# widgital/python-audio-tools

Hardware: AMD Instinct MI355X
Metric: FLAC-8 encode frames/s (4096-sample 44.1k stereo) at 1/2/4/8 GPUs; bit-exact (higher is better)
Workload: dtype int32 residuals / f64 LPC analysis (s16 PCM in); 1 GPU; FLAC-8 batch encode, 1024 tracks x 64 frames x 4096 samples per GPU, 44.1 kHz 16-bit stereo, PCM and .flac images in HBM; tracks_per_gpu=1024, frames_per_track=64, block_size=4096, preset=FLAC-8 (-l 12 -m -e -R 6), parallelism=dp1 (tracks sharded per GPU, weak scaling)

## Files before the change

### python-audio-tools_amd/csrc/engine.hip

```cpp
#include "handle_lock.h"
#include "host_common.h"
#include <hip/hip_runtime.h>

#include <sched.h>

#include <algorithm>
#include <array>
#include <cmath>
#include <condition_variable>
#include <cstdio>
#include <cstdlib>
#include <cstring>
#include <deque>
#include <functional>
#include <future>
#include <map>
#include <memory>
#include <mutex>
#include <string>
#include <thread>
#include <vector>

#include "../../include/atgpu.h"
#include "crc_common.h"
#include "flac_dev.h"
#include "launch.h"
#include "md5_cpu.h"
#include "ogg_demux.h"
#include "ogg_mux.h"

namespace {

thread_local ErrSlot g_err;
#define HIP_TRY(expr) ATG_HIP_TRY(g_err, expr, #expr)

const char kVendor[] = "Python Audio Tools 2.22alpha1";

const int kNumTimed = 8;
const char *kTimedNames[kNumTimed] = {"lpc_analyze", "subframe_search", "frame_decide",
                                      "track_scan",  "frame_pack",      "track_md5",
                                      "stream_header", "total"};
const char *kOggTimedNames[4] = {"ogg_plan", "ogg_pages", "ogg_split", "ogg_crc"};

void build_crc_tables(uint32_t t16[4][256], uint32_t *t8, uint16_t adv[24][16],
                      uint16_t advq[kCrcQ][6][16])
{
    crc_build_tables<16>(0x8005u, &t16[0][0], 4);
    crc_build_tables<8>(0x07u, t8, 1);
    crc_build_advance<16>(t16[0], &adv[0][0], 24);
    for (int i = 0; i < 16; ++i)
        advq[0][0][i] = adv[2][i];
    for (int q = 1; q < kCrcQ; ++q)
        for (int i = 0; i < 16; ++i)
            advq[q][0][i] = (uint16_t)crc_advance<16>(adv[2], advq[q - 1][0][i]);
    for (int q = 0; q < kCrcQ; ++q)
        for (int s = 1; s < 6; ++s)
            crc_square<16>(advq[q][s - 1], advq[q][s]);
}

}

namespace {
struct Plan;
struct HostJob;
}

struct EncSlot {
    DevBuf frames, tracks, order, coef, shift, est, sub, fdesc, tout, err;
    DevBuf rice_big, scratch;
    DevBuf slow;
    hipStream_t s_aux = nullptr;
    hipEvent_t ev[2 * kNumTimed] = {};
    hipEvent_t ev_tables = nullptr, ev_pack = nullptr, ev_done = nullptr;
    std::shared_ptr<Plan> plan;
    const Plan *uploaded = nullptr;
    hipEvent_t ev_reuse = nullptr;
    bool reuse_pending = false;
    TrackOut *tout_h = nullptr;
    size_t tout_cap = 0;
    FrameDesc *fdesc_h = nullptr;
    size_t fdesc_cap = 0;
    uint32_t *err_h = nullptr;
    size_t err_cap = 0;
    bool want_fdesc = false;
    bool end_pending = false;
    const void *pend_pcm = nullptr;
    int pend_fmt = 0;
    uint8_t *pend_out = nullptr;
    bool pend_split = false;
    atg_status end_status = ATG_OK;
    std::string end_error;
    bool md5_host = false;
    uint8_t *hpcm = nullptr;
    size_t hpcm_cap = 0;
    DevBuf dpack;
    uint8_t *hmd5 = nullptr;
    size_t hmd5_cap = 0;
    DevBuf md5in;
    hipEvent_t ev_hpcm = nullptr;
    std::vector<std::future<void>> hash_jobs;
    bool rolled = false;
    uint32_t roll_parts = 0, roll_done = 0;
    bool busy = false;
    bool done = false;
    bool host = false;
    uint64_t ticket = 0;
    atg_status status = ATG_OK;
    std::string error;
    float times[kNumTimed] = {};
};



constexpr uint64_t kEncSlots = 3;
constexpr uint64_t kMaxSlots = 32;
static_assert(kMaxSlots <= kRollMax, "one rolled launch covers every slot");
constexpr uint64_t kRollMinDepth = 4;

constexpr uint64_t kHostStages = kEncSlots + 1;

constexpr size_t kResultCopy = 8192;

struct HostStage {
    DevBuf d_pcm, d_img, d_pack, d_off;
    uint8_t *p_in = nullptr, *p_out = nullptr;
    size_t p_in_cap = 0, p_out_cap = 0;
    uint64_t *p_off = nullptr;
    size_t p_off_cap = 0;
    hipEvent_t ev_h2d = nullptr;
    hipEvent_t ev_packed = nullptr;
    hipEvent_t ev_d2h = nullptr;
};

struct HashPool {
    std::vector<std::thread> th;
    std::mutex mu;
    std::condition_variable cv;
    std::deque<std::packaged_task<void()>> q;
    bool stop = false;
    explicit HashPool(unsigned n)
    {
        for (unsigned i = 0; i < n; ++i)
            th.emplace_back([this] {
                for (;;) {
                    std::packaged_task<void()> job;
                    {
                        std::unique_lock<std::mutex> lk(mu);
                        cv.wait(lk, [this] { return stop || !q.empty(); });
                        if (q.empty())
                            return;
                        job = std::move(q.front());
                        q.pop_front();
                    }
                    job();
                }
            });
    }
    std::future<void> submit(std::function<void()> f)
    {
        std::packaged_task<void()> job(std::move(f));
        std::future<void> fut = job.get_future();
        {
            std::lock_guard<std::mutex> lk(mu);
            q.push_back(std::move(job));
        }
        cv.notify_one();
        return fut;
    }
    ~HashPool()
    {
        {
            std::lock_guard<std::mutex> lk(mu);
            stop = true;
        }
        cv.notify_all();
        for (std::thread &t : th)
            t.join();
    }
};

struct atg_engine {
    std::recursive_mutex mu;
    int device = 0;
    uint32_t flags = 0;
    std::unique_ptr<HashPool> pool;
    bool sync_call = false;
    hipStream_t s_main = nullptr;
    hipStream_t s_pack = nullptr;
    EncSlot slot[kMaxSlots];
    uint64_t depth = kEncSlots;
    bool depth_user = false;
    hipStream_t s_md5 = nullptr;
    std::deque<EncSlot *> roll_q;
    DevBuf windows;
    HostStage hs[kHostStages];
    hipStream_t s_h2d = nullptr, s_d2h = nullptr;
    hipStream_t s_hpack = nullptr;
    uint64_t chunk_bytes = 512ull << 20;
    std::deque<std::unique_ptr<HostJob>> hjobs;
    std::deque<std::pair<HostJob *, size_t>> hflight;
    HostJob *hcopy_job = nullptr;
    size_t hcopy_chunk = 0;
    uint64_t hseq = 0;
    uint64_t next_hjob = 1;
    std::map<uint32_t, uint32_t> win_off;
    std::vector<double> win_host;
    size_t win_uploaded = 0;
    hipEvent_t ev_win = nullptr;
    float times[kNumTimed] = {};
    bool have_times = false;
    uint64_t next_ticket = 1;
    std::vector<uint8_t> plan_key;
    std::shared_ptr<Plan> plan_cached;
    DevBuf ogg_stage, ogg_tmpl, ogg_hp, ogg_trk, ogg_frm, ogg_pgoff, ogg_out, ogg_pages;
    DevBuf ogg_pcm, ogg_img;
    const uint32_t *ogg_crc = nullptr, *ogg_adv = nullptr;
    hipEvent_t ogg_ev[5] = {};
    float ogg_times[4] = {};
    bool ogg_last = false;
};

namespace {

struct Plan {
    FlacParams p;
    std::vector<FrameInfo> frames;
    std::vector<TrackInfo> tracks;
    std::vector<uint32_t> track_frame_pos;
    std::vector<uint32_t> order;
    uint64_t frame_bound = 0;
    uint64_t out_bytes = 0;
    uint32_t n_reg_prefix = 0;
    bool big = false;
    uint32_t big_nmax = 0;
    uint32_t big_porder = 0;
    bool frames_only = false;
};

const uint32_t kBigGrid = 1024;

uint64_t big_row_bytes(const Plan &pl) { return ((uint64_t)pl.big_nmax * 4u + 255u) & ~255ull; }

uint64_t big_slot_bytes(const Plan &pl)
{
    return big_row_bytes(pl) + (16ull << pl.big_porder);
}

uint32_t qlp_precision_for(uint32_t n)
{
    return n <= 192 ? 7 : n <= 384 ? 8 : n <= 576 ? 9 : n <= 1152 ? 10 : n <= 2304 ? 11
         : n <= 4608 ? 12 : 13;
}

atg_status make_plan(const atg_flac_options *o, const atg_track *tracks, uint32_t n_tracks,
                     uint32_t channels, uint32_t bps, uint32_t rate, Plan &pl,
                     bool frames_only = false, uint32_t index_base = 0,
                     const uint32_t *index_bases = nullptr)
{
    if (!o)
        return g_err.fail(ATG_ERR_INVALID, "options is NULL");
    if (channels < 1 || channels > 8)
        return g_err.fail(ATG_ERR_INVALID, "channels must be 1..8");
    if (bps < 4 || bps > 24)
        return g_err.fail(ATG_ERR_UNSUPPORTED, "bits_per_sample must be 4..24 on the GPU path");
    if (o->block_size == 0)
        return g_err.fail(ATG_ERR_INVALID, "block_size must be > 0");
    if (o->block_size > ATG_BIG_MAX_BLOCK)
        return g_err.fail(ATG_ERR_UNSUPPORTED, "block_size > 65535 cannot be framed");
    if (o->max_lpc_order > ATG_MAX_LPC)
        return g_err.fail(ATG_ERR_INVALID, "max_lpc_order must be <= 32");
    if (o->max_residual_partition_order > ATG_BIG_MAX_PORDER)
        return g_err.fail(ATG_ERR_INVALID, "max_residual_partition_order must be <= 15");
    if (o->padding_size > 0xFFFFFFu)
        return g_err.fail(ATG_ERR_INVALID, "padding_size must fit in 24 bits");
    if (rate == 0)
        return g_err.fail(ATG_ERR_INVALID, "sample_rate must be > 0");
    FlacParams &p = pl.p;
    std::memset(&p, 0, sizeof(p));
    p.block_size = o->block_size;
    p.max_lpc_order = o->max_lpc_order;
    p.max_porder = o->max_residual_partition_order;
    p.qlp_precision = qlp_precision_for(o->block_size);
    p.max_rice = bps <= 16 ? 14 : 30;
    p.mid_side = o->mid_side != 0;
    p.adaptive_mid_side = o->adaptive_mid_side != 0;
    p.exhaustive = o->exhaustive_model_search != 0;
    p.try_verbatim = !o->disable_verbatim_subframes;
    p.try_constant = !o->disable_constant_subframes;
    p.try_fixed = !o->disable_fixed_subframes;
    p.try_lpc = !(o->disable_lpc_subframes || o->max_lpc_order == 0);
    p.channels = channels;
    p.bps = bps;
    p.sample_rate = rate;
    p.n_cand = (channels == 2 && (p.mid_side || p.adaptive_mid_side)) ? 4 : channels;
    p.n_tracks = n_tracks;
    const uint32_t M = p.max_lpc_order;
    p.coef_row = std::max<uint32_t>(2, (M + 1u) & ~1u);
    p.coef_stride = std::max<uint32_t>(1, M) * p.coef_row;
    p.padding_size = o->padding_size;
    p.header_bytes = frames_only ? 0u : 4 + 4 + 34 + 4 + 4 + 29 + 4 + 4 + o->padding_size;
    pl.frames_only = frames_only;

    const uint64_t B = o->block_size;
    const uint64_t nsub = channels;

    pl.tracks.resize(n_tracks);
    std::vector<uint32_t> lens;
    std::vector<uint32_t> owner;
    for (uint32_t t = 0; t < n_tracks; ++t) {
        const atg_track &tr = tracks[t];
        TrackInfo &ti = pl.tracks[t];
        ti.pcm_start = tr.pcm_offset;
        ti.pcm_frames = tr.pcm_frames;
        ti.first_pos = (uint32_t)lens.size();
        if (tr.frame_sizes) {
            uint64_t sum = 0;
            for (uint64_t k = 0; k < tr.n_frame_sizes; ++k) {
                const uint32_t n = tr.frame_sizes[k];
                if (n == 0 || n > ATG_BIG_MAX_BLOCK)
                    return g_err.fail(n ? ATG_ERR_UNSUPPORTED : ATG_ERR_INVALID,
                                "explicit frame sizes must be 1..65535");
                sum += n;
                lens.push_back(n);
                owner.push_back(t);
            }
            if (sum != tr.pcm_frames)
                return g_err.fail(ATG_ERR_INVALID, "frame sizes do not sum to pcm_frames");
        } else {
            for (uint64_t done = 0; done < tr.pcm_frames; done += B) {
                lens.push_back((uint32_t)std::min<uint64_t>(B, tr.pcm_frames - done));
                owner.push_back(t);
            }
        }
        ti.n_frames = (uint32_t)(lens.size() - ti.first_pos);
        if (lens.size() > 0x7FFFFFFFull)
            return g_err.fail(ATG_ERR_INVALID, "too many frames in one batch");
    }
    const size_t nfr = lens.size();
    pl.order.resize(nfr);
    pl.frames.resize(nfr);
    pl.track_frame_pos.resize(n_tracks);
    size_t n_full = 0;
    for (size_t i = 0; i < nfr; ++i)
        n_full += lens[i] == B ? 1 : 0;
    size_t id_full = 0, id_other = n_full;
    std::vector<uint64_t> start(n_tracks, 0);
    std::vector<uint32_t> idx(n_tracks, 0);
    for (size_t i = 0; i < nfr; ++i) {
        const uint32_t t = owner[i];
        const size_t id = lens[i] == B ? id_full++ : id_other++;
        pl.order[i] = (uint32_t)id;
        FrameInfo &f = pl.frames[id];
        f.pcm_start = pl.tracks[t].pcm_start + start[t];
        f.n = lens[i];
        f.track = t;
        f.index = (index_bases ? index_bases[t] : index_base) + idx[t]++;
        f.win_off = 0;
        start[t] += lens[i];
    }
    uint32_t maxn = 0;
    for (size_t i = 0; i < nfr; ++i)
        maxn = std::max(maxn, lens[i]);
    const uint64_t nb = std::max<uint64_t>(B, maxn);
    uint64_t fb = 16 + nsub * ((8 + 32 + nb * (bps + 1) + 7) / 8) + 2;
    pl.big = nb > ATG_MAX_BLOCK || p.max_porder > ATG_MAX_PORDER;
    if (!p.try_verbatim)
        fb = pl.big ? 2 * fb + 120 * 1024 : std::max<uint64_t>(fb, 120 * 1024);
    pl.frame_bound = fb;
    p.frame_bound = (uint32_t)fb;
    p.frame_lds_words = (uint32_t)((fb + 3) / 4 + 2);
    if (!pl.big && p.frame_lds_words * 4ull > 128 * 1024)
        return g_err.fail(ATG_ERR_UNSUPPORTED, "frame image exceeds the pack kernel's LDS budget");
    if (pl.big) {
        pl.big_nmax = maxn;
        pl.big_porder = 0;
        for (size_t i = 0; i < nfr; ++i) {
            const uint32_t tz = (uint32_t)__builtin_ctz(lens[i]);
            pl.big_porder = std::max(pl.big_porder, std::min<uint32_t>(p.max_porder, tz));
        }
    }
    uint64_t out = 0;
    for (uint32_t t = 0; t < n_tracks; ++t) {
        TrackInfo &ti = pl.tracks[t];
        pl.track_frame_pos[t] = ti.first_pos;
        ti.out_base = out;
        out += p.header_bytes + (uint64_t)ti.n_frames * fb;
        out = (out + 15) & ~15ull;
    }
    p.n_frames = (uint32_t)pl.frames.size();
    pl.out_bytes = out;
    pl.n_reg_prefix = 0;
    if (channels == 2 && p.n_cand == 4 && bps <= 16 && B == ATG_MAX_BLOCK && !pl.big)
        while (pl.n_reg_prefix < p.n_frames && pl.frames[pl.n_reg_prefix].n == ATG_MAX_BLOCK &&
               (pl.frames[pl.n_reg_prefix].pcm_start & 3u) == 0)
            pl.n_reg_prefix++;
    return ATG_OK;
}

void tukey(uint32_t N, double *w)
{
    const double alpha = 0.5;
    const unsigned window1 = (unsigned)(alpha * (N - 1)) / 2;
    const unsigned window2 = (unsigned)((N - 1) * (1.0 - (alpha / 2.0)));
    for (unsigned n = 0; n < N; n++) {
        if (n <= window1)
            w[n] = 0.5 * (1.0 + std::cos(M_PI * (((2 * n) / (alpha * (N - 1))) - 1.0)));
        else if (n <= window2)
            w[n] = 1.0;
        else
            w[n] = 0.5 * (1.0 + std::cos(M_PI * (((2.0 * n) / (alpha * (N - 1))) -
                                                 (2.0 / alpha) + 1.0)));
    }
}

atg_status prepare_windows(atg_engine *e, Plan &pl, hipStream_t s)
{
    if (!pl.p.try_lpc)
        return ATG_OK;
    const uint32_t M = pl.p.max_lpc_order;
    for (FrameInfo &f : pl.frames) {
        if (f.n <= M + 1)
            continue;
        auto it = e->win_off.find(f.n);
        if (it == e->win_off.end()) {
            const uint32_t off = (uint32_t)e->win_host.size();
            e->win_host.resize(off + f.n);
            tukey(f.n, e->win_host.data() + off);
            it = e->win_off.emplace(f.n, off).first;
        }
        f.win_off = it->second;
    }
    if (e->win_host.size() != e->win_uploaded) {
        const size_t need = e->win_host.size() * sizeof(double) + 64;
        if (need > e->windows.cap && e->windows.p)
            HIP_TRY(hipDeviceSynchronize());
        HIP_TRY(e->windows.ensure(need));
        HIP_TRY(hipMemcpyAsync(e->windows.p, e->win_host.data(),
                               e->win_host.size() * sizeof(double), hipMemcpyHostToDevice,
                               s));
        e->win_uploaded = e->win_host.size();
        if (!e->ev_win)
            HIP_TRY(hipEventCreateWithFlags(&e->ev_win, hipEventDisableTiming));
        HIP_TRY(hipEventRecord(e->ev_win, s));
    } else if (e->ev_win) {
        HIP_TRY(hipStreamWaitEvent(s, e->ev_win, 0));
    }
    return ATG_OK;
}

void par_memcpy(void *dst, const void *src, size_t n, unsigned nt)
{
    const size_t kMin = 8u << 20;
    if (n < kMin || nt < 2) {
        std::memcpy(dst, src, n);
        return;
    }
    nt = (unsigned)std::min<size_t>(nt, n / (kMin / 4));
    std::vector<std::thread> th;
    const size_t part = (n / nt + 4095) & ~(size_t)4095;
    for (unsigned i = 0; i < nt; ++i) {
        const size_t a = (size_t)i * part;
        if (a >= n)
            break;
        const size_t len = std::min(part, n - a);
        th.emplace_back([=] { std::memcpy((uint8_t *)dst + a, (const uint8_t *)src + a, len); });
    }
    for (auto &t : th)
        t.join();
}

bool is_pinned(const void *p)
{
    if (!p)
        return false;
    hipPointerAttribute_t a;
    if (hipPointerGetAttributes(&a, p) != hipSuccess) {
        (void)hipGetLastError();
        return false;
    }
    return a.type == hipMemoryTypeHost;
}

template <class T>
hipError_t ensure_pinned(T *&p, size_t &cap, size_t n)
{
    if (p && n <= cap)
        return hipSuccess;
    if (p)
        (void)hipHostFree(p);
    p = nullptr;
    cap = 0;
    const size_t want = std::max<size_t>(n, 16);
    hipError_t e = hipHostMalloc((void **)&p, want * sizeof(T), hipHostMallocDefault);
    if (e == hipSuccess)
        cap = want;
    return e;
}

atg_status batch_end_queue(atg_engine *e, EncSlot &sl, hipEvent_t after);

atg_status batch_end(atg_engine *e, EncSlot &sl, hipEvent_t after)
{
    sl.end_pending = false;
    const atg_status st = batch_end_queue(e, sl, after);
    if (st != ATG_OK) {
        sl.end_status = st;
        sl.end_error = g_err.msg;
    }
    return st;
}

atg_status batch_end_queue(atg_engine *e, EncSlot &sl, hipEvent_t after)
{
    const Plan &pl = *sl.plan;
    const FlacParams &p = pl.p;
    const size_t nf = pl.frames.size(), nt = pl.tracks.size();
    const TrackInfo *dtr = (const TrackInfo *)sl.tracks.p;
    TrackOut *dto = (TrackOut *)sl.tout.p;
    uint32_t *derr = (uint32_t *)sl.err.p;
    hipEvent_t *ev = sl.ev;
    hipStream_t q = sl.rolled ? e->s_md5 : sl.s_aux;
    if (sl.rolled) {
        if (!pl.frames_only)
            HIP_TRY(launch_track_md5_finish(p, sl.pend_pcm, sl.pend_fmt, dtr, dto, q));
    } else if (sl.pend_split && !pl.frames_only) {
        if (after)
            HIP_TRY(hipStreamWaitEvent(q, after, 0));
        HIP_TRY(launch_track_md5(p, sl.pend_pcm, sl.pend_fmt, dtr, dto, 1, q));
    }
    HIP_TRY(hipEventRecord(ev[2 * 5 + 1], q));
    HIP_TRY(hipStreamWaitEvent(q, sl.ev_pack, 0));
    HIP_TRY(hipEventRecord(ev[12], q));
    if (!pl.frames_only)
        HIP_TRY(launch_stream_header(p, dtr, dto, sl.pend_out, q));
    HIP_TRY(hipEventRecord(ev[13], q));
    HIP_TRY(hipEventRecord(ev[15], q));
    for (size_t o = 0, nb = nt * sizeof(TrackOut); o < nb; o += kResultCopy)
        HIP_TRY(hipMemcpyAsync((uint8_t *)sl.tout_h + o, (const uint8_t *)dto + o,
                               std::min<size_t>(kResultCopy, nb - o), hipMemcpyDeviceToHost, q));
    if (sl.want_fdesc && nf)
        HIP_TRY(hipMemcpyAsync(sl.fdesc_h, sl.fdesc.p, nf * sizeof(FrameDesc),
                               hipMemcpyDeviceToHost, q));
    HIP_TRY(hipMemcpyAsync(sl.err_h, derr, sizeof(uint32_t), hipMemcpyDeviceToHost, q));
    HIP_TRY(hipEventRecord(sl.ev_done, q));
    return ATG_OK;
}

atg_status ensure_aux_stream(EncSlot &sl);

atg_status ensure_roll_streams(atg_engine *e)
{
    if (e->s_md5)
        return ATG_OK;
    int prio_lo = 0, prio_hi = 0;
    HIP_TRY(hipDeviceGetStreamPriorityRange(&prio_lo, &prio_hi));
    HIP_TRY(hipStreamCreateWithPriority(&e->s_md5, hipStreamNonBlocking, prio_hi));
    return ATG_OK;
}

atg_status roll_step(atg_engine *e, hipEvent_t after, EncSlot *only)
{
    MdRollArgs a;
    std::memset(&a, 0, sizeof(a));
    std::vector<EncSlot *> starting, finished;
    uint32_t wg = 0;
    for (EncSlot *sl : e->roll_q) {
        if (only && sl != only)
            continue;
        const FlacParams &p = sl->plan->p;
        MdRollBatch &b = a.b[a.n++];
        b.pcm = sl->pend_pcm;
        b.tracks = (const TrackInfo *)sl->tracks.p;
        b.tout = (TrackOut *)sl->tout.p;
        b.n_tracks = p.n_tracks;
        b.channels = p.channels;
        b.bps = p.bps;
        b.fmt = (uint32_t)sl->pend_fmt;
        b.wg0 = wg;
        b.parts = sl->roll_parts;
        b.part = sl->roll_done;
        b.part_end = only ? sl->roll_parts : sl->roll_done + 1u;
        wg += (p.n_tracks + 63u) / 64u;
        if (b.part == 0)
            starting.push_back(sl);
        sl->roll_done = b.part_end;
        if (sl->roll_done == sl->roll_parts)
            finished.push_back(sl);
    }
    if (!a.n)
        return ATG_OK;
    if (after)
        HIP_TRY(hipStreamWaitEvent(e->s_md5, after, 0));
    for (EncSlot *sl : starting)
        HIP_TRY(hipEventRecord(sl->ev[2 * 5], e->s_md5));
    HIP_TRY(launch_track_md5_roll(a, e->s_md5));
    for (EncSlot *sl : finished) {
        e->roll_q.erase(std::find(e->roll_q.begin(), e->roll_q.end(), sl));
        const atg_status st = batch_end(e, *sl, nullptr);
        if (st != ATG_OK)
            return st;
    }
    return ATG_OK;
}

void drain_slot(atg_engine *e, EncSlot &sl)
{
    (void)hipStreamSynchronize(e->s_main);
    for (hipStream_t q : {e->s_pack, e->s_md5, sl.s_aux})
        if (q)
            (void)hipStreamSynchronize(q);
}

unsigned host_hash_threads()
{
    unsigned n = std::max(1u, std::thread::hardware_concurrency());
    cpu_set_t cs;
    if (sched_getaffinity(0, sizeof(cs), &cs) == 0)
        n = std::max(1, CPU_COUNT(&cs));
    if (FILE *f = std::fopen("/sys/fs/cgroup/cpu.max", "r")) {
        char q[32] = {0};
        unsigned long per = 0;
        if (std::fscanf(f, "%31s %lu", q, &per) == 2 && std::strcmp(q, "max") != 0 && per)
            n = std::min<unsigned>(n, std::max(1ul, std::strtoul(q, nullptr, 10) / per));
        std::fclose(f);
    }
    return std::min(n, 32u);
}

constexpr size_t kHashGroup = md5cpu::kMultiLanes;

bool want_host_md5(atg_engine *e, const Plan &pl, int fmt, bool md5_early)
{
    const FlacParams &p = pl.p;
    if (pl.frames_only || md5_early || p.bps < 8 || p.bps % 8 || pl.tracks.empty())
        return false;
    if (e->flags & ATG_ENGINE_MD5_GPU)
        return false;
    if (e->flags & ATG_ENGINE_MD5_HOST)
        return true;
    const uint64_t bb = p.bps / 8, cs = fmt == ATG_PCM_S16 ? 2 : 4;
    uint64_t maxb = 0, tot = 0;
    for (const TrackInfo &t : pl.tracks) {
        const uint64_t b = t.pcm_frames * p.channels * bb;
        maxb = std::max(maxb, b);
        tot += b;
    }
    (void)cs;
    const double gpu_ms = (double)maxb / 64.0 * 0.8e-3;
    const unsigned th = host_hash_threads();
    const uint64_t groups = (pl.tracks.size() + kHashGroup - 1) / kHashGroup;
    const double hash_ms = md5cpu::multi_simd()
                               ? (double)tot / (double)std::min<uint64_t>(th, groups) / 6e6
                               : (double)tot / (th * 450e3);
    const double host_ms = hash_ms + (double)tot / 40e6;
    return gpu_ms > 40.0 && host_ms < gpu_ms;
}

atg_status start_host_md5(atg_engine *e, EncSlot &sl, const Plan &pl, const void *d_pcm, int fmt)
{
    const FlacParams &p = pl.p;
    const size_t nt = pl.tracks.size();
    const uint64_t cs = fmt == ATG_PCM_S16 ? 2 : 4;
    const uint32_t bb = p.bps / 8;
    for (std::future<void> &f : sl.hash_jobs)
        f.wait();
    sl.hash_jobs.clear();
    std::vector<uint64_t> off(nt), len(nt);
    uint64_t total = 0;
    for (size_t t = 0; t < nt; ++t) {
        len[t] = pl.tracks[t].pcm_frames * p.channels * bb;
        off[t] = total;
        total += (len[t] + 15u) & ~15ull;
    }
    HIP_TRY(ensure_pinned(sl.hpcm, sl.hpcm_cap, (size_t)std::max<uint64_t>(total, 1)));
    HIP_TRY(ensure_pinned(sl.hmd5, sl.hmd5_cap, 16 * nt));
    HIP_TRY(sl.md5in.ensure(16 * nt));
    HIP_TRY(sl.dpack.ensure((size_t)std::max<uint64_t>(total, 1)));
    if (!sl.ev_hpcm)
        HIP_TRY(hipEventCreateWithFlags(&sl.ev_hpcm, hipEventDisableTiming));
    for (size_t t = 0; t < nt; ++t) {
        const TrackInfo &ti = pl.tracks[t];
        HIP_TRY(launch_md5_pack((const uint8_t *)d_pcm + ti.pcm_start * p.channels * cs,
                                fmt == ATG_PCM_S16, ti.pcm_frames * p.channels, bb,
                                (uint8_t *)sl.dpack.p + off[t], sl.s_aux));
    }
    if (total)
        HIP_TRY(hipMemcpyAsync(sl.hpcm, sl.dpack.p, total, hipMemcpyDeviceToHost, sl.s_aux));
    HIP_TRY(hipEventRecord(sl.ev_hpcm, sl.s_aux));
    if (!e->pool)
        e->pool.reset(new HashPool(host_hash_threads()));
    const hipEvent_t ev = sl.ev_hpcm;
    for (size_t g0 = 0; g0 < nt; g0 += kHashGroup) {
        const int n = (int)std::min<size_t>(kHashGroup, nt - g0);
        std::array<const uint8_t *, kHashGroup> src{};
        std::array<uint64_t, kHashGroup> bytes{};
        for (int i = 0; i < n; ++i) {
            src[i] = sl.hpcm + off[g0 + i];
            bytes[i] = len[g0 + i];
        }
        uint8_t(*dst)[16] = (uint8_t(*)[16])(sl.hmd5 + 16 * g0);
        sl.hash_jobs.push_back(e->pool->submit([=] {
            (void)hipEventSynchronize(ev);
            md5cpu::hash_bytes_multi(src.data(), bytes.data(), n, dst);
        }));
    }
    return ATG_OK;
}

atg_status finish_host_md5(EncSlot &sl)
{
    for (std::future<void> &f : sl.hash_jobs)
        f.wait();
    sl.hash_jobs.clear();
    const size_t nt = sl.plan->tracks.size();
    if (nt) {
        HIP_TRY(hipMemcpyAsync(sl.md5in.p, sl.hmd5, 16 * nt, hipMemcpyHostToDevice, sl.s_aux));
        HIP_TRY(launch_put_md5((TrackOut *)sl.tout.p, (const uint8_t *)sl.md5in.p, (uint32_t)nt,
                               sl.s_aux));
    }
    return ATG_OK;
}

atg_status enqueue_batch(atg_engine *e, EncSlot &sl, const std::shared_ptr<Plan> &plp,
                         const void *d_pcm, int fmt, uint8_t *d_out, uint64_t out_cap,
                         bool want_fdesc, hipEvent_t wait_before = nullptr, bool pipelined = false,
                         bool md5_early = false)
{
    Plan &pl = *plp;
    FlacParams &p = pl.p;
    if (pl.out_bytes > out_cap)
// ... 1659 lines not shown
```

### python-audio-tools_amd/csrc/flac_lpc.hip

```cpp
#include <hip/hip_runtime.h>
#include <math.h>
#include <stdint.h>

#include "flac_dev.h"
#include "launch.h"
#include "pcm_read.h"
#include "residual.h"
#include "wave.h"

#pragma clang fp contract(off)


__device__ __forceinline__ int32_t d2i_x86(double x)
{
    if (!(x > -2147483649.0 && x < 2147483648.0))
        return INT32_MIN;
    return (int32_t)x;
}

template <int LAGS>
__device__ __forceinline__ void quantize_store(const double (&lp)[LAGS],
                                               int order, int prec,
                                               int16_t *__restrict__ q, uint32_t row,
                                               int8_t *__restrict__ shift_out)
{
    double l = 2.2250738585072014e-308;
#pragma unroll
    for (int i = 0; i < LAGS; ++i) {
        if (i < order) {
            const double a = fabs(lp[i]);
            l = a > l ? a : l;
        }
    }
    int log2cmax;
    frexp(l, &log2cmax);
    int shift = (prec - 1) - (log2cmax - 1) - 1;
    shift = shift < -16 ? -16 : shift;
    shift = shift > 15 ? 15 : shift;
    const int qmax = (1 << (prec - 1)) - 1;
    const int qmin = -(1 << (prec - 1));
    double err = 0.0;
#pragma unroll
    for (int i = 0; i < LAGS; ++i) {
        if (i < order) {
            if (shift >= 0)
                err += lp[i] * (double)(1 << shift);
            else
                err += lp[i] / (double)(1 << -shift);
            const int32_t ei = d2i_x86(round(err));
            q[i] = (int16_t)(ei < qmin ? qmin : (ei > qmax ? qmax : ei));
            err -= (double)ei;
        }
    }
    for (uint32_t i = (uint32_t)order; i < row; ++i)
        q[i] = 0;
    *shift_out = (int8_t)(shift >= 0 ? shift : 0);
}

template <int MODE, typename T, int K>
__device__ __forceinline__ void autocorr(const T *__restrict__ src, const double *__restrict__ win,
                                         uint32_t ch, uint32_t cand, uint32_t n_loop,
                                         uint32_t nlast, uint32_t n_max, double (&acc)[K],
                                         double (&hist)[K])
{
    int32_t sv[K];
    double wv[K];
#pragma unroll
    for (int u = 0; u < K; ++u) {
        const uint32_t j = min((uint32_t)u, nlast);
        sv[u] = cand_at<MODE>(src, j, ch, cand);
        wv[u] = win[j];
    }
    for (uint32_t j0 = 0; j0 < n_max; j0 += K) {
        double xv[K];
#pragma unroll
        for (int u = 0; u < K; ++u)
            xv[u] = (j0 + (uint32_t)u < n_loop) ? (double)sv[u] * wv[u] : 0.0;
#pragma unroll
        for (int u = 0; u < K; ++u) {
            const uint32_t j = min(j0 + K + (uint32_t)u, nlast);
            sv[u] = cand_at<MODE>(src, j, ch, cand);
            wv[u] = win[j];
        }
#pragma unroll
        for (int u = 0; u < K; ++u) {
            const double x = xv[u];
            hist[u] = x;
#pragma unroll
            for (int L = 0; L < K; ++L) {
                const double prod = hist[(u - L + K) % K] * x;
                acc[L] = acc[L] + prod;
            }
        }
    }
}

template <int K, bool VEC4>
__device__ __forceinline__ void autocorr_ms16(const uint32_t *__restrict__ pairs,
                                              const double *__restrict__ win, uint32_t cand,
                                              uint32_t N, double (&acc)[K], double (&hist)[K])
{
    const uint32_t wts = cand == 0u ? 0x00000001u : cand == 1u ? 0x00010000u
                       : cand == 2u ? 0x00010001u : 0xFFFF0001u;
    const int gsh = cand == 2u ? 1 : 0;
    const uint32_t nfull = N / K * K;
    uint32_t j0 = 0;
    if (VEC4) {
        const uint4 *__restrict__ q4 = (const uint4 *)pairs;
        for (; j0 + 4u * K <= N; j0 += 4u * K) {
            uint32_t pv[4 * K];
#pragma unroll
            for (int i = 0; i < K; ++i) {
                const uint4 v = q4[(j0 >> 2) + (uint32_t)i];
                pv[4 * i] = v.x;
                pv[4 * i + 1] = v.y;
                pv[4 * i + 2] = v.z;
                pv[4 * i + 3] = v.w;
            }
#pragma unroll
            for (int i = 0; i < 4 * K; ++i)
                asm volatile("" : "+v"(pv[i]));
#pragma unroll
            for (int sub = 0; sub < 4; ++sub) {
                double xv[K];
#pragma unroll
                for (int u = 0; u < K; ++u) {
                    const int v = __builtin_amdgcn_sdot2(
                        __builtin_bit_cast(short2_t, pv[sub * K + u]),
                        __builtin_bit_cast(short2_t, wts), 0, false);
                    xv[u] = (double)(v >> gsh) * win[j0 + (uint32_t)(sub * K + u)];
                }
#pragma unroll
                for (int u = 0; u < K; ++u) {
                    const double x = xv[u];
                    hist[u] = x;
#pragma unroll
                    for (int L = 0; L < K; ++L) {
                        const double prod = hist[(u - L + K) % K] * x;
                        acc[L] = acc[L] + prod;
                    }
                }
            }
        }
    }
    for (; j0 < nfull; j0 += K) {
        double xv[K];
#pragma unroll
        for (int u = 0; u < K; ++u) {
            const int v = __builtin_amdgcn_sdot2(__builtin_bit_cast(short2_t, pairs[j0 + u]),
                                                 __builtin_bit_cast(short2_t, wts), 0, false);
            xv[u] = (double)(v >> gsh) * win[j0 + u];
        }
#pragma unroll
        for (int u = 0; u < K; ++u) {
            const double x = xv[u];
            hist[u] = x;
#pragma unroll
            for (int L = 0; L < K; ++L) {
                const double prod = hist[(u - L + K) % K] * x;
                acc[L] = acc[L] + prod;
            }
        }
    }
    if (j0 < N) {
        double xv[K];
#pragma unroll
        for (int u = 0; u < K; ++u) {
            const uint32_t j = min(j0 + (uint32_t)u, N - 1u);
            const int v = __builtin_amdgcn_sdot2(__builtin_bit_cast(short2_t, pairs[j]),
                                                 __builtin_bit_cast(short2_t, wts), 0, false);
            xv[u] = j0 + (uint32_t)u < N ? (double)(v >> gsh) * win[j] : 0.0;
        }
#pragma unroll
        for (int u = 0; u < K; ++u) {
            const double x = xv[u];
            hist[u] = x;
#pragma unroll
            for (int L = 0; L < K; ++L) {
                const double prod = hist[(u - L + K) % K] * x;
                acc[L] = acc[L] + prod;
            }
        }
    }
}

template <typename T, int LAGS>
__global__ __launch_bounds__(64) void k_lpc_analyze(
    FlacParams p, const T *__restrict__ pcm,
    const FrameInfo *__restrict__ frames, const double *__restrict__ windows,
    int16_t *__restrict__ coef_tab, int8_t *__restrict__ shift_tab,
    uint8_t *__restrict__ est_tab)
{
    constexpr int K = LAGS + 1;
    const uint32_t fpw = 64u / p.n_cand;
    const uint32_t fl = threadIdx.x / p.n_cand;
    const uint32_t cand = threadIdx.x - fl * p.n_cand;
    const uint32_t f = blockIdx.x * fpw + fl;
    const bool ms = (p.n_cand == 4u) && (p.channels == 2u);
    const bool active = fl < fpw && f < p.n_frames;
    const FrameInfo fi = frames[active ? f : 0u];
    const int M = (int)p.max_lpc_order;
    const uint32_t N = active ? fi.n : 0u;
    const bool do_lpc = active && N > (uint32_t)M + 1u;
    const uint32_t n_loop = do_lpc ? N : 0u;
    const uint32_t n_max = wave_max_u32(n_loop);
    if (n_max == 0u)
        return;

    double acc[K];
    double hist[K];
#pragma unroll
    for (int k = 0; k < K; ++k) {
        acc[k] = 0.0;
        hist[k] = 0.0;
    }
    const double *__restrict__ win = windows + fi.win_off;
    const T *__restrict__ src = pcm + fi.pcm_start * p.channels;
    const uint32_t nlast = n_loop ? n_loop - 1u : 0u;
    const int mode = pcm_mode(pcm, ms);
    const uint32_t n_first = uniform_u32(do_lpc ? N : 0u);
    const bool uniform_n = wave_all(!active || (do_lpc ? N : 0u) == n_first) && n_first > 0u;
    if (mode == PCM_MS16 && uniform_n) {
        const double *__restrict__ wu =
            windows + uniform_u32(active ? fi.win_off : 0u);
        const bool al16 = wave_all(((uintptr_t)src & 15u) == 0u);
        if (al16)
            autocorr_ms16<K, true>((const uint32_t *)src, wu, cand, n_first, acc, hist);
        else
            autocorr_ms16<K, false>((const uint32_t *)src, wu, cand, n_first, acc, hist);
    } else switch (mode) {
    case PCM_MS16:
        autocorr<PCM_MS16, T, K>(src, win, p.channels, cand, n_loop, nlast, n_max, acc, hist);
        break;
    case PCM_MS:
        autocorr<PCM_MS, T, K>(src, win, p.channels, cand, n_loop, nlast, n_max, acc, hist);
        break;
    default:
        autocorr<PCM_CH, T, K>(src, win, p.channels, cand, n_loop, nlast, n_max, acc, hist);
    }
    if (!do_lpc)
        return;

    const size_t sub = (size_t)f * p.n_cand + cand;
    int16_t *__restrict__ qout = coef_tab + sub * p.coef_stride;
    int8_t *__restrict__ sout = shift_tab + sub * (size_t)M;
    const int prec = (int)p.qlp_precision;

    double prev[LAGS], cur[LAGS], errv[LAGS];
#pragma unroll
    for (int k = 0; k < LAGS; ++k) {
        prev[k] = 0.0;
        cur[k] = 0.0;
        errv[k] = 0.0;
    }
    double k0 = acc[1] / acc[0];
    cur[0] = k0;
    errv[0] = acc[0] * (1.0 - (k0 * k0));
    quantize_store<LAGS>(cur, 1, prec, qout, p.coef_row, sout);
#pragma unroll
    for (int i = 1; i < LAGS; ++i) {
        if (i < M) {
#pragma unroll
            for (int j = 0; j < LAGS; ++j)
                prev[j] = cur[j];
            double q = acc[i + 1];
#pragma unroll
            for (int j = 0; j < LAGS; ++j)
                if (j < i)
                    q -= (prev[j] * acc[i - j]);
            const double kk = q / errv[i - 1];
#pragma unroll
            for (int j = 0; j < LAGS; ++j)
                if (j < i)
                    cur[j] = prev[j] - (kk * prev[i - j - 1]);
            cur[i] = kk;
            errv[i] = errv[i - 1] * (1.0 - (kk * kk));
            quantize_store<LAGS>(cur, i + 1, prec, qout + i * p.coef_row, p.coef_row,
                                 sout + i);
        }
    }

    if (!p.exhaustive) {
        const double ln2 = 0.69314718055994530942;
        const double error_scale = (ln2 * ln2) / ((double)N * 2.0);
        int best = 0;
        double best_bits = 1.7976931348623157e308;
        bool done = false;
#pragma unroll
        for (int i = 0; i < LAGS; ++i) {
            if (i < M && !done) {
                const int order = i + 1;
                if (errv[i] > 0.0) {
                    const unsigned header = (unsigned)order * (p.bps + p.qlp_precision);
                    double bpr = log(errv[i] * error_scale) / (ln2 * 2);
                    bpr = bpr > 0.0 ? bpr : 0.0;
                    const double est = (double)header + bpr * (double)(N - (unsigned)order);
                    if (est < best_bits) {
                        best = order;
                        best_bits = est;
                    }
                } else {
                    best = order;
                    done = true;
                }
            }
        }
        est_tab[sub] = (uint8_t)best;
    }
}

template <typename T, int LAGS>
static hipError_t launch_t(const FlacParams &p, const T *pcm, const FrameInfo *frames,
                           const double *windows, int16_t *coef_tab,
                           int8_t *shift_tab, uint8_t *est_tab, hipStream_t s)
{
    const uint32_t fpw = 64u / p.n_cand;
    dim3 grid((p.n_frames + fpw - 1u) / fpw);
    hipLaunchKernelGGL((k_lpc_analyze<T, LAGS>), grid, dim3(64), 0, s, p, pcm,
                       frames, windows, coef_tab, shift_tab, est_tab);
    return hipGetLastError();
}

template <typename T>
static hipError_t launch_lags(const FlacParams &p, const T *pcm,
                              const FrameInfo *frames, const double *windows,
                              int16_t *coef_tab, int8_t *shift_tab,
                              uint8_t *est_tab, hipStream_t s)
{
    const uint32_t M = p.max_lpc_order;
    if (M <= 8)
        return launch_t<T, 8>(p, pcm, frames, windows, coef_tab, shift_tab, est_tab, s);
    if (M <= 12)
        return launch_t<T, 12>(p, pcm, frames, windows, coef_tab, shift_tab, est_tab, s);
    return launch_t<T, ATG_MAX_LPC>(p, pcm, frames, windows, coef_tab, shift_tab,
                                    est_tab, s);
}

hipError_t launch_lpc_analyze(const FlacParams &p, const void *pcm, int fmt,
                              const FrameInfo *frames, const double *windows,
                              int16_t *coef_tab, int8_t *shift_tab,
                              uint8_t *est_tab, hipStream_t s)
{
    if (p.max_lpc_order == 0 || !p.try_lpc || p.n_frames == 0)
        return hipSuccess;
    if (fmt == 0)
        return launch_lags<int16_t>(p, (const int16_t *)pcm, frames, windows,
                                    coef_tab, shift_tab, est_tab, s);
    return launch_lags<int32_t>(p, (const int32_t *)pcm, frames, windows,
                                coef_tab, shift_tab, est_tab, s);
}
```

Before: 8.620 million frames/s.

## Skip window multiply and fuse autocorrelation FMAs inside flat Tukey window region

The host now records, in a slot just before each window, the contiguous range where the Tukey window equals 1.0. Inside that range the autocorrelation kernels skip the window load and multiply and accumulate with FMA instead of a separate multiply and add. This holds bit-exactly only when the products of integer samples are exact in double, which the LPC_FMA_MAX_BITS check on bps is meant to guarantee. The cost is extra per-group branching and a shifted window layout.

```diff
diff --git a/python-audio-tools_amd/csrc/engine.hip b/python-audio-tools_amd/csrc/engine.hip
--- a/python-audio-tools_amd/csrc/engine.hip
+++ b/python-audio-tools_amd/csrc/engine.hip
@@ -25,6 +25,7 @@
 #include "crc_common.h"
 #include "flac_dev.h"
 #include "launch.h"
+#include "lpc_flat.h"
 #include "md5_cpu.h"
 #include "ogg_demux.h"
 #include "ogg_mux.h"
@@ -423,9 +424,12 @@
             continue;
         auto it = e->win_off.find(f.n);
         if (it == e->win_off.end()) {
-            const uint32_t off = (uint32_t)e->win_host.size();
+            const uint32_t off = (uint32_t)e->win_host.size() + 1u;
             e->win_host.resize(off + f.n);
             tukey(f.n, e->win_host.data() + off);
+            const WinFlat wf = window_flat_run(e->win_host.data() + off, f.n);
+            static_assert(sizeof(WinFlat) == sizeof(double), "WinFlat fills one window slot");
+            memcpy(e->win_host.data() + off - 1, &wf, sizeof wf);
             it = e->win_off.emplace(f.n, off).first;
         }
         f.win_off = it->second;
diff --git a/python-audio-tools_amd/csrc/flac_lpc.hip b/python-audio-tools_amd/csrc/flac_lpc.hip
--- a/python-audio-tools_amd/csrc/flac_lpc.hip
+++ b/python-audio-tools_amd/csrc/flac_lpc.hip
@@ -4,6 +4,7 @@
 
 #include "flac_dev.h"
 #include "launch.h"
+#include "lpc_flat.h"
 #include "pcm_read.h"
 #include "residual.h"
 #include "wave.h"
@@ -60,8 +61,8 @@
 template <int MODE, typename T, int K>
 __device__ __forceinline__ void autocorr(const T *__restrict__ src, const double *__restrict__ win,
                                          uint32_t ch, uint32_t cand, uint32_t n_loop,
-                                         uint32_t nlast, uint32_t n_max, double (&acc)[K],
-                                         double (&hist)[K])
+                                         uint32_t nlast, uint32_t n_max, uint2 flat,
+                                         double (&acc)[K], double (&hist)[K])
 {
     int32_t sv[K];
     double wv[K];
@@ -71,34 +72,38 @@
         sv[u] = cand_at<MODE>(src, j, ch, cand);
         wv[u] = win[j];
     }
+    bool fused = false;
     for (uint32_t j0 = 0; j0 < n_max; j0 += K) {
         double xv[K];
 #pragma unroll
-        for (int u = 0; u < K; ++u)
-            xv[u] = (j0 + (uint32_t)u < n_loop) ? (double)sv[u] * wv[u] : 0.0;
+        for (int u = 0; u < K; ++u) {
+            const bool in = j0 + (uint32_t)u < n_loop;
+            if (fused)
+                xv[u] = in ? (double)sv[u] : 0.0;
+            else
+                xv[u] = in ? (double)sv[u] * wv[u] : 0.0;
+        }
+        const bool fused_next = wave_all(n_loop == 0u || group_flat<K>(j0 + K, flat.x, flat.y));
 #pragma unroll
         for (int u = 0; u < K; ++u) {
             const uint32_t j = min(j0 + K + (uint32_t)u, nlast);
             sv[u] = cand_at<MODE>(src, j, ch, cand);
-            wv[u] = win[j];
-        }
-#pragma unroll
-        for (int u = 0; u < K; ++u) {
-            const double x = xv[u];
-            hist[u] = x;
-#pragma unroll
-            for (int L = 0; L < K; ++L) {
-                const double prod = hist[(u - L + K) % K] * x;
-                acc[L] = acc[L] + prod;
-            }
-        }
+            if (!fused_next)
+                wv[u] = win[j];
+        }
+        if (fused)
+            chains<true>(xv, acc, hist);
+        else
+            chains<false>(xv, acc, hist);
+        fused = fused_next;
     }
 }
 
 template <int K, bool VEC4>
 __device__ __forceinline__ void autocorr_ms16(const uint32_t *__restrict__ pairs,
                                               const double *__restrict__ win, uint32_t cand,
-                                              uint32_t N, double (&acc)[K], double (&hist)[K])
+                                              uint32_t N, uint2 flat, double (&acc)[K],
+                                              double (&hist)[K])
 {
     const uint32_t wts = cand == 0u ? 0x00000001u : cand == 1u ? 0x00010000u
                        : cand == 2u ? 0x00010001u : 0xFFFF0001u;
@@ -123,44 +128,40 @@
 #pragma unroll
             for (int sub = 0; sub < 4; ++sub) {
                 double xv[K];
+                const bool fused = group_flat<K>(j0 + (uint32_t)(sub * K), flat.x, flat.y);
 #pragma unroll
                 for (int u = 0; u < K; ++u) {
                     const int v = __builtin_amdgcn_sdot2(
                         __builtin_bit_cast(short2_t, pv[sub * K + u]),
                         __builtin_bit_cast(short2_t, wts), 0, false);
-                    xv[u] = (double)(v >> gsh) * win[j0 + (uint32_t)(sub * K + u)];
+                    if (fused)
+                        xv[u] = (double)(v >> gsh);
+                    else
+                        xv[u] = (double)(v >> gsh) * win[j0 + (uint32_t)(sub * K + u)];
                 }
-#pragma unroll
-                for (int u = 0; u < K; ++u) {
-                    const double x = xv[u];
-                    hist[u] = x;
-#pragma unroll
-                    for (int L = 0; L < K; ++L) {
-                        const double prod = hist[(u - L + K) % K] * x;
-                        acc[L] = acc[L] + prod;
-                    }
-                }
+                if (fused)
+                    chains<true>(xv, acc, hist);
+                else
+                    chains<false>(xv, acc, hist);
             }
         }
     }
     for (; j0 < nfull; j0 += K) {
         double xv[K];
+        const bool fused = group_flat<K>(j0, flat.x, flat.y);
 #pragma unroll
         for (int u = 0; u < K; ++u) {
             const int v = __builtin_amdgcn_sdot2(__builtin_bit_cast(short2_t, pairs[j0 + u]),
                                                  __builtin_bit_cast(short2_t, wts), 0, false);
-            xv[u] = (double)(v >> gsh) * win[j0 + u];
-        }
-#pragma unroll
-        for (int u = 0; u < K; ++u) {
-            const double x = xv[u];
-            hist[u] = x;
-#pragma unroll
-            for (int L = 0; L < K; ++L) {
-                const double prod = hist[(u - L + K) % K] * x;
-                acc[L] = acc[L] + prod;
-            }
-        }
+            if (fused)
+                xv[u] = (double)(v >> gsh);
+            else
+                xv[u] = (double)(v >> gsh) * win[j0 + u];
+        }
+        if (fused)
+            chains<true>(xv, acc, hist);
+        else
+            chains<false>(xv, acc, hist);
     }
     if (j0 < N) {
         double xv[K];
@@ -171,16 +172,7 @@
                                                  __builtin_bit_cast(short2_t, wts), 0, false);
             xv[u] = j0 + (uint32_t)u < N ? (double)(v >> gsh) * win[j] : 0.0;
         }
-#pragma unroll
-        for (int u = 0; u < K; ++u) {
-            const double x = xv[u];
-            hist[u] = x;
-#pragma unroll
-            for (int L = 0; L < K; ++L) {
-                const double prod = hist[(u - L + K) % K] * x;
-                acc[L] = acc[L] + prod;
-            }
-        }
+        chains<false>(xv, acc, hist);
     }
 }
 
@@ -220,23 +212,32 @@
     const int mode = pcm_mode(pcm, ms);
     const uint32_t n_first = uniform_u32(do_lpc ? N : 0u);
     const bool uniform_n = wave_all(!active || (do_lpc ? N : 0u) == n_first) && n_first > 0u;
+    uint2 flat = make_uint2(0u, 0u);
+    if (do_lpc && p.bps + 1u <= (uint32_t)LPC_FMA_MAX_BITS) {
+        const WinFlat wf = *(const WinFlat *)(win - 1);
+        flat = make_uint2(wf.lo, wf.hi);
+    }
     if (mode == PCM_MS16 && uniform_n) {
         const double *__restrict__ wu =
             windows + uniform_u32(active ? fi.win_off : 0u);
+        const uint2 fu = make_uint2(uniform_u32(flat.x), uniform_u32(flat.y));
         const bool al16 = wave_all(((uintptr_t)src & 15u) == 0u);
         if (al16)
-            autocorr_ms16<K, true>((const uint32_t *)src, wu, cand, n_first, acc, hist);
+            autocorr_ms16<K, true>((const uint32_t *)src, wu, cand, n_first, fu, acc, hist);
         else
-            autocorr_ms16<K, false>((const uint32_t *)src, wu, cand, n_first, acc, hist);
+            autocorr_ms16<K, false>((const uint32_t *)src, wu, cand, n_first, fu, acc, hist);
     } else switch (mode) {
     case PCM_MS16:
-        autocorr<PCM_MS16, T, K>(src, win, p.channels, cand, n_loop, nlast, n_max, acc, hist);
+        autocorr<PCM_MS16, T, K>(src, win, p.channels, cand, n_loop, nlast, n_max, flat, acc,
+                                 hist);
         break;
     case PCM_MS:
-        autocorr<PCM_MS, T, K>(src, win, p.channels, cand, n_loop, nlast, n_max, acc, hist);
+        autocorr<PCM_MS, T, K>(src, win, p.channels, cand, n_loop, nlast, n_max, flat, acc,
+                                 hist);
         break;
     default:
-        autocorr<PCM_CH, T, K>(src, win, p.channels, cand, n_loop, nlast, n_max, acc, hist);
+        autocorr<PCM_CH, T, K>(src, win, p.channels, cand, n_loop, nlast, n_max, flat, acc,
+                                 hist);
     }
     if (!do_lpc)
         return;
diff --git a/python-audio-tools_amd/csrc/lpc_flat.h b/python-audio-tools_amd/csrc/lpc_flat.h
--- /dev/null
+++ b/python-audio-tools_amd/csrc/lpc_flat.h
@@ -0,0 +1,58 @@
+#pragma once
+
+#include <stdint.h>
+
+#if defined(__HIPCC__)
+#include <hip/hip_runtime.h>
+#define LPC_HD __host__ __device__ __forceinline__
+#else
+#define LPC_HD inline
+#endif
+
+#define LPC_FMA_MAX_BITS 26
+
+struct WinFlat {
+    uint32_t lo;
+    uint32_t hi;
+};
+
+inline WinFlat window_flat_run(const double *w, uint32_t N)
+{
+    uint32_t lo = 0, hi = 0, ones = 0;
+    for (uint32_t n = 0; n < N; n++) {
+        if (w[n] == 1.0) {
+            if (!ones)
+                lo = n;
+            hi = n + 1;
+            ones++;
+        }
+    }
+    if (hi - lo != ones)
+        lo = hi = 0;
+    return WinFlat{lo, hi};
+}
+
+template <int K>
+LPC_HD bool group_flat(uint32_t j0, uint32_t lo, uint32_t hi)
+{
+    return j0 >= lo + (uint32_t)(K - 1) && j0 + (uint32_t)K <= hi;
+}
+
+template <bool FUSED, int K>
+LPC_HD void chains(const double (&xv)[K], double (&acc)[K], double (&hist)[K])
+{
+#pragma unroll
+    for (int u = 0; u < K; ++u) {
+        const double x = xv[u];
+        hist[u] = x;
+#pragma unroll
+        for (int L = 0; L < K; ++L) {
+            if (FUSED) {
+                acc[L] = __builtin_fma(hist[(u - L + K) % K], x, acc[L]);
+            } else {
+                const double prod = hist[(u - L + K) % K] * x;
+                acc[L] = acc[L] + prod;
+            }
+        }
+    }
+}
```

After: 8.684 million frames/s, median of 6. No clear change (+0.7%).
